# lucidrains/progen

Measured on NVIDIA H100. Metric: tokens_per_sec, higher is better.
Workload: dtype bf16

## Files before the change

progen_b200/csrc/attn_wgmma.cu:

```cuda
#include <cuda.h>
#include "common.cuh"
#include "tc_ptx.cuh"
#include "../../include/progen_b200.h"

namespace {

using namespace tc;

constexpr int DH = 64;
constexpr int TILE = 64;
constexpr int TILE_BYTES = TILE * DH * 2;
constexpr float LOG2E = 1.4426950408889634f;
constexpr float LN2 = 0.6931471805599453f;
constexpr int SMEM_BYTES = 1024  + 2 * TILE_BYTES + 2 * 2 * TILE_BYTES + 64;

struct Dims {
  int n, w, h;
  const float* rot_sin;
  const float* rot_cos;
};

__device__ __forceinline__ float quad_max(float v) {
  v = fmaxf(v, __shfl_xor_sync(0xffffffffu, v, 1));
  return fmaxf(v, __shfl_xor_sync(0xffffffffu, v, 2));
}
__device__ __forceinline__ float quad_sum(float v) {
  v += __shfl_xor_sync(0xffffffffu, v, 1);
  return v + __shfl_xor_sync(0xffffffffu, v, 2);
}
__device__ __forceinline__ uint32_t unrotate_pack(const Dims& dm, int pos, int jj, float d0, float d1) {
  if (dm.rot_sin) {
    const float s = __ldg(dm.rot_sin + pos * (DH / 2) + jj), c = __ldg(dm.rot_cos + pos * (DH / 2) + jj);
    const float a = d0 * c + d1 * s, b = d1 * c - d0 * s;
    d0 = a; d1 = b;
  }
  return pack_bf16x2(d0, d1);
}
template <int R> __device__ __forceinline__ void zero(float (&a)[R]) {
#pragma unroll
  for (int i = 0; i < R; ++i) a[i] = 0.f;
}
__device__ __forceinline__ void acc_to_a(uint32_t (&a)[4][4], const float (&s)[32]) {
#pragma unroll
  for (int kk = 0; kk < 4; ++kk)
#pragma unroll
    for (int i = 0; i < 4; ++i) a[kk][i] = pack_bf16x2(s[8 * kk + 2 * i], s[8 * kk + 2 * i + 1]);
}
__device__ __forceinline__ void issue_a_xt(float (&acc)[32], uint32_t a, uint32_t x) {
#pragma unroll
  for (int kk = 0; kk < 4; ++kk) wgmma_m64n64k16_ss<0>(acc, make_smem_desc<false>(a + 32 * kk), make_smem_desc<false>(x + 32 * kk));
}
__device__ __forceinline__ void issue_p_x(float (&acc)[32], const uint32_t (&p)[4][4], uint32_t x) {
#pragma unroll
  for (int kk = 0; kk < 4; ++kk) wgmma_m64n64k16_rs<1>(acc, p[kk], make_smem_desc<true>(x + 2048 * kk));
}
template <int R> __device__ __forceinline__ void mma_begin(float (&acc)[R]) {
  fence_regs(acc);
  wgmma_fence();
}
template <int R> __device__ __forceinline__ void mma_end(float (&acc)[R]) {
  wgmma_commit();
  wgmma_wait<0>();
  fence_regs(acc);
}

struct Smem {
  uint32_t fixed0, fixed1, ring, bars;
  __device__ Smem(uint8_t* raw) {
    fixed0 = (smem_u32(raw) + 1023u) & ~1023u;
    fixed1 = fixed0 + TILE_BYTES;
    ring = fixed1 + TILE_BYTES;
    bars = ring + 4 * TILE_BYTES;
  }
  __device__ uint32_t a(int st) const { return ring + st * 2 * TILE_BYTES; }
  __device__ uint32_t b(int st) const { return a(st) + TILE_BYTES; }
  __device__ uint32_t fixed_bar() const { return bars; }
  __device__ uint32_t full(int st) const { return bars + 8 + 8 * st; }
};

__device__ __forceinline__ void init_bars(const Smem& sm) {
  if (threadIdx.x == 0) {
    mbar_init(sm.fixed_bar(), 1);
    mbar_init(sm.full(0), 1);
    mbar_init(sm.full(1), 1);
    fence_barrier_init();
  }
  __syncthreads();
}

__global__ void __launch_bounds__(128) attn_fwd_wgmma_kernel(const __grid_constant__ CUtensorMap tm_qkv, bf16* __restrict__ out,
                                                             float* __restrict__ lse, const Dims dm) {
  extern __shared__ uint8_t smem_raw[];
  const Smem sm(smem_raw);
  const int tid = threadIdx.x, lane = tid & 31, warp = tid >> 5;
  const int g = lane >> 2, t4 = lane & 3;
  const int b = blockIdx.z, hh = blockIdx.y;
  const int q0 = blockIdx.x * TILE, win = q0 / dm.w, i0 = q0 % dm.w;
  const int I = dm.h * DH;
  const int row0 = b * dm.n;
  const int nprev = win > 0 ? dm.w / TILE : 0;
  const int ntiles = nprev + (i0 + TILE) / TILE;
  auto key_pos = [&](int kt) { return kt < nprev ? (win - 1) * dm.w + kt * TILE : win * dm.w + (kt - nprev) * TILE; };
  auto issue = [&](int kt, int st) {
    mbar_expect_tx(sm.full(st), 2 * TILE_BYTES);
    tma_load_2d(sm.a(st), &tm_qkv, sm.full(st), I + hh * DH, row0 + key_pos(kt));
    tma_load_2d(sm.b(st), &tm_qkv, sm.full(st), 2 * I + hh * DH, row0 + key_pos(kt));
  };
  init_bars(sm);
  if (tid == 0) {
    prefetch_tensormap(&tm_qkv);
    mbar_expect_tx(sm.fixed_bar(), TILE_BYTES);
    tma_load_2d(sm.fixed0, &tm_qkv, sm.fixed_bar(), hh * DH, row0 + q0);
    for (int kt = 0; kt < 2 && kt < ntiles; ++kt) issue(kt, kt);
  }

  const float sc = 0.125f  * LOG2E;
  float m_run[2], l_run[2];
  m_run[0] = m_run[1] = (win == 0) ? 0.f : -INFINITY;
  l_run[0] = l_run[1] = (win == 0) ? (float)dm.w : 0.f;
  float o[32];
  zero(o);
  const int qi_lo = i0 + warp * 16;
  mbar_wait(sm.fixed_bar(), 0);

  for (int kt = 0; kt < ntiles; ++kt) {
    const int st = kt & 1;
    mbar_wait(sm.full(st), (kt >> 1) & 1);
    float s[32];
    zero(s);
    mma_begin(s);
    issue_a_xt(s, sm.fixed0, sm.a(st));
    mma_end(s);
    const int c0 = (kt - nprev) * TILE;
    const bool need_mask = kt >= nprev && c0 + TILE - 1 > qi_lo;
    float tmax[2] = {-INFINITY, -INFINITY};
#pragma unroll
    for (int i = 0; i < 32; ++i) {
      float v = s[i] * sc;
      if (need_mask) {
        const int kj = c0 + 8 * (i >> 2) + 2 * t4 + (i & 1);
        const int qi = qi_lo + g + (((i >> 1) & 1) << 3);
        if (kj > qi) v = -INFINITY;
      }
      s[i] = v;
      tmax[(i >> 1) & 1] = fmaxf(tmax[(i >> 1) & 1], v);
    }
    float corr[2], rsum[2] = {0.f, 0.f};
#pragma unroll
    for (int r = 0; r < 2; ++r) {
      const float mn = fmaxf(m_run[r], quad_max(tmax[r]));
      corr[r] = exp2f(m_run[r] - mn);
      m_run[r] = mn;
    }
#pragma unroll
    for (int i = 0; i < 32; ++i) {
      const float p = exp2f(s[i] - m_run[(i >> 1) & 1]);
      s[i] = p;
      rsum[(i >> 1) & 1] += p;
    }
#pragma unroll
    for (int r = 0; r < 2; ++r) l_run[r] = l_run[r] * corr[r] + quad_sum(rsum[r]);
#pragma unroll
    for (int i = 0; i < 32; ++i) o[i] *= corr[(i >> 1) & 1];
    uint32_t pa[4][4];
    acc_to_a(pa, s);
    mma_begin(o);
    issue_p_x(o, pa, sm.b(st));
    mma_end(o);
    __syncthreads();
    if (tid == 0 && kt + 2 < ntiles) {
      fence_proxy_async();
      issue(kt + 2, st);
    }
  }
#pragma unroll
  for (int r = 0; r < 2; ++r) {
    const long long t = (long long)row0 + q0 + warp * 16 + g + 8 * r;
    const float inv = 1.f / l_run[r];
    bf16* op = out + t * I + hh * DH + 2 * t4;
#pragma unroll
    for (int j = 0; j < 8; ++j)
      *reinterpret_cast<uint32_t*>(op + 8 * j) = pack_bf16x2(o[4 * j + 2 * r] * inv, o[4 * j + 2 * r + 1] * inv);
    if (t4 == 0) lse[t * dm.h + hh] = m_run[r] * LN2 + logf(l_run[r]);
  }
}

__global__ void __launch_bounds__(128) attn_bwd_dq_wgmma_kernel(const __grid_constant__ CUtensorMap tm_qkv,
                                                                const __grid_constant__ CUtensorMap tm_do,
                                                                const bf16* __restrict__ out, const bf16* __restrict__ dout,
                                                                const float* __restrict__ lse, float* __restrict__ delta,
                                                                bf16* __restrict__ dqkv, const Dims dm) {
  extern __shared__ uint8_t smem_raw[];
  const Smem sm(smem_raw);
  const int tid = threadIdx.x, lane = tid & 31, warp = tid >> 5;
  const int g = lane >> 2, t4 = lane & 3;
  const int b = blockIdx.z, hh = blockIdx.y;
  const int q0 = blockIdx.x * TILE, win = q0 / dm.w, i0 = q0 % dm.w;
  const int I = dm.h * DH;
  const long long ld = 3LL * I;
  const int row0 = b * dm.n;
  const int nprev = win > 0 ? dm.w / TILE : 0;
  const int ntiles = nprev + (i0 + TILE) / TILE;
  auto key_pos = [&](int kt) { return kt < nprev ? (win - 1) * dm.w + kt * TILE : win * dm.w + (kt - nprev) * TILE; };
  auto issue = [&](int kt, int st) {
    mbar_expect_tx(sm.full(st), 2 * TILE_BYTES);
    tma_load_2d(sm.a(st), &tm_qkv, sm.full(st), I + hh * DH, row0 + key_pos(kt));
    tma_load_2d(sm.b(st), &tm_qkv, sm.full(st), 2 * I + hh * DH, row0 + key_pos(kt));
  };
  init_bars(sm);
  if (tid == 0) {
    prefetch_tensormap(&tm_qkv);
    prefetch_tensormap(&tm_do);
    mbar_expect_tx(sm.fixed_bar(), 2 * TILE_BYTES);
    tma_load_2d(sm.fixed0, &tm_qkv, sm.fixed_bar(), hh * DH, row0 + q0);
    tma_load_2d(sm.fixed1, &tm_do, sm.fixed_bar(), hh * DH, row0 + q0);
    for (int kt = 0; kt < 2 && kt < ntiles; ++kt) issue(kt, kt);
  }

  const float scale = 0.125f ;
  const float sc = scale * LOG2E;
  float L2[2], Dl[2];
#pragma unroll
  for (int r = 0; r < 2; ++r) {
    const long long t = (long long)row0 + q0 + warp * 16 + g + 8 * r;
    L2[r] = lse[t * dm.h + hh] * LOG2E;
    float acc = 0.f;
#pragma unroll
    for (int j = 0; j < 8; ++j) {
      const uint32_t ov = *reinterpret_cast<const uint32_t*>(out + t * I + hh * DH + 8 * j + 2 * t4);
      const uint32_t dv = *reinterpret_cast<const uint32_t*>(dout + t * I + hh * DH + 8 * j + 2 * t4);
      const float2 fo = __bfloat1622float2(*reinterpret_cast<const __nv_bfloat162*>(&ov));
      const float2 fd = __bfloat1622float2(*reinterpret_cast<const __nv_bfloat162*>(&dv));
      acc += fo.x * fd.x + fo.y * fd.y;
    }
    Dl[r] = quad_sum(acc);
    if (t4 == 0) delta[t * dm.h + hh] = Dl[r];
  }
  float dq[32];
  zero(dq);
  const int qi_lo = i0 + warp * 16;
  mbar_wait(sm.fixed_bar(), 0);

  for (int kt = 0; kt < ntiles; ++kt) {
    const int st = kt & 1;
    mbar_wait(sm.full(st), (kt >> 1) & 1);
    float s[32], dp[32];
    zero(s);
    zero(dp);
    fence_regs(dp);
    mma_begin(s);
    issue_a_xt(s, sm.fixed0, sm.a(st));
    issue_a_xt(dp, sm.fixed1, sm.b(st));
    mma_end(s);
    fence_regs(dp);
    const int c0 = (kt - nprev) * TILE;
    const bool need_mask = kt >= nprev && c0 + TILE - 1 > qi_lo;
#pragma unroll
    for (int i = 0; i < 32; ++i) {
      const int r = (i >> 1) & 1;
      float p = exp2f(s[i] * sc - L2[r]);
      if (need_mask) {
        const int kj = c0 + 8 * (i >> 2) + 2 * t4 + (i & 1);
        const int qi = qi_lo + g + (r << 3);
        if (kj > qi) p = 0.f;
      }
      s[i] = p * (dp[i] - Dl[r]) * scale;
    }
    uint32_t dsa[4][4];
    acc_to_a(dsa, s);
    mma_begin(dq);
    issue_p_x(dq, dsa, sm.a(st));
    mma_end(dq);
    __syncthreads();
    if (tid == 0 && kt + 2 < ntiles) {
      fence_proxy_async();
      issue(kt + 2, st);
    }
  }
#pragma unroll
  for (int r = 0; r < 2; ++r) {
    const int pos = q0 + warp * 16 + g + 8 * r;
    bf16* op = dqkv + ((long long)row0 + pos) * ld + hh * DH + 2 * t4;
#pragma unroll
    for (int j = 0; j < 8; ++j)
      *reinterpret_cast<uint32_t*>(op + 8 * j) = unrotate_pack(dm, pos, 4 * j + t4, dq[4 * j + 2 * r], dq[4 * j + 2 * r + 1]);
  }
}

__global__ void __launch_bounds__(128) attn_bwd_dkv_wgmma_kernel(const __grid_constant__ CUtensorMap tm_qkv,
                                                                 const __grid_constant__ CUtensorMap tm_do,
                                                                 const float* __restrict__ lse, const float* __restrict__ delta,
                                                                 bf16* __restrict__ dqkv, const Dims dm) {
  extern __shared__ uint8_t smem_raw[];
  const Smem sm(smem_raw);
  const int tid = threadIdx.x, lane = tid & 31, warp = tid >> 5;
  const int g = lane >> 2, t4 = lane & 3;
  const int b = blockIdx.z, hh = blockIdx.y;
  const int k0 = blockIdx.x * TILE, win = k0 / dm.w, j0 = k0 % dm.w;
  const int I = dm.h * DH;
  const long long ld = 3LL * I;
  const int row0 = b * dm.n;
  const int nwin = dm.n / dm.w;
  const int nown = (dm.w - j0) / TILE;
  const int nnext = (win + 1 < nwin) ? dm.w / TILE : 0;
  const int ntiles = nown + nnext;
  auto q_pos = [&](int qt) { return qt < nown ? win * dm.w + j0 + qt * TILE : (win + 1) * dm.w + (qt - nown) * TILE; };
  auto issue = [&](int qt, int st) {
    mbar_expect_tx(sm.full(st), 2 * TILE_BYTES);
    tma_load_2d(sm.a(st), &tm_qkv, sm.full(st), hh * DH, row0 + q_pos(qt));
    tma_load_2d(sm.b(st), &tm_do, sm.full(st), hh * DH, row0 + q_pos(qt));
  };
  init_bars(sm);
  if (tid == 0) {
    prefetch_tensormap(&tm_qkv);
    prefetch_tensormap(&tm_do);
    mbar_expect_tx(sm.fixed_bar(), 2 * TILE_BYTES);
    tma_load_2d(sm.fixed0, &tm_qkv, sm.fixed_bar(), I + hh * DH, row0 + k0);
    tma_load_2d(sm.fixed1, &tm_qkv, sm.fixed_bar(), 2 * I + hh * DH, row0 + k0);
    for (int qt = 0; qt < 2 && qt < ntiles; ++qt) issue(qt, qt);
  }

  const float scale = 0.125f ;
  const float sc = scale * LOG2E;
  float dk[32], dv[32];
  zero(dk);
  zero(dv);
  const int kj_lo = j0 + warp * 16;
  mbar_wait(sm.fixed_bar(), 0);

  for (int qt = 0; qt < ntiles; ++qt) {
    const int st = qt & 1;
    const int qp = q_pos(qt);
    float Lq[16], Dq[16];
#pragma unroll
    for (int j = 0; j < 8; ++j)
#pragma unroll
      for (int c = 0; c < 2; ++c) {
        const long long t = (long long)row0 + qp + 8 * j + 2 * t4 + c;
        Lq[2 * j + c] = __ldg(lse + t * dm.h + hh) * LOG2E;
        Dq[2 * j + c] = __ldg(delta + t * dm.h + hh);
      }
    mbar_wait(sm.full(st), (qt >> 1) & 1);
    float s[32], dp[32];
    zero(s);
    zero(dp);
    fence_regs(dp);
    mma_begin(s);
    issue_a_xt(s, sm.fixed0, sm.a(st));
    issue_a_xt(dp, sm.fixed1, sm.b(st));
    mma_end(s);
    fence_regs(dp);
    const bool own = qt < nown;
    const int c0 = j0 + qt * TILE;
    const bool need_mask = own && c0 < kj_lo + 15;
#pragma unroll
    for (int i = 0; i < 32; ++i) {
      const int col = 8 * (i >> 2) + 2 * t4 + (i & 1);
      const int ci = 2 * (i >> 2) + (i & 1);
      float p = exp2f(s[i] * sc - Lq[ci]);
      if (need_mask) {
        const int qi = c0 + col;
        const int kj = kj_lo + g + (((i >> 1) & 1) << 3);
        if (kj > qi) p = 0.f;
      }
      dp[i] = p * (dp[i] - Dq[ci]) * scale;
      s[i] = p;
    }
    uint32_t pa[4][4], dsa[4][4];
    acc_to_a(pa, s);
    acc_to_a(dsa, dp);
    fence_regs(dk);
    mma_begin(dv);
    issue_p_x(dv, pa, sm.b(st));
    issue_p_x(dk, dsa, sm.a(st));
    mma_end(dv);
    fence_regs(dk);
    __syncthreads();
    if (tid == 0 && qt + 2 < ntiles) {
      fence_proxy_async();
      issue(qt + 2, st);
    }
  }
#pragma unroll
  for (int r = 0; r < 2; ++r) {
    const int pos = k0 + warp * 16 + g + 8 * r;
    bf16* pk = dqkv + ((long long)row0 + pos) * ld + I + hh * DH + 2 * t4;
    bf16* pv = pk + I;
#pragma unroll
    for (int j = 0; j < 8; ++j) {
      *reinterpret_cast<uint32_t*>(pk + 8 * j) = unrotate_pack(dm, pos, 4 * j + t4, dk[4 * j + 2 * r], dk[4 * j + 2 * r + 1]);
      *reinterpret_cast<uint32_t*>(pv + 8 * j) = unrotate_pack(dm, pos, 4 * j + t4, dv[4 * j + 2 * r], dv[4 * j + 2 * r + 1]);
    }
  }
}

template <typename K> int prepare(K kern) {
  static bool done = false;
  if (!done) {
    PG_CUDA(cudaFuncSetAttribute(kern, cudaFuncAttributeMaxDynamicSharedMemorySize, SMEM_BYTES));
    done = true;
  }
  return PROGEN_OK;
}

int check_dims(const void* qkv, int B, int seq_len, int window, int heads, int dim_head, bool full_windows) {
  PG_CHECK_ARG(qkv != nullptr && B > 0 && heads > 0 && dim_head == DH && window % TILE == 0 && seq_len > 0 &&
               seq_len % (full_windows ? window : TILE) == 0);
  PG_CHECK_ARG((long long)B * seq_len < (1ll << 31));
  return PROGEN_OK;
}

}

extern "C" {

int progen_local_attn_fwd_tc(const void* qkv, void* out, float* lse, int B, int seq_len, int window, int heads, int dim_head,
                             void* stream) {
  int rc = check_dims(qkv, B, seq_len, window, heads, dim_head, false);
  if (rc) return rc;
  const int I = heads * DH;
  const uint64_t T = (uint64_t)B * seq_len;
  CUtensorMap tm;
  if ((rc = pg_tensor_map_2d_bf16(qkv, 3ull * I, T, 3ull * I, DH, TILE, &tm))) return rc;
  if ((rc = prepare(attn_fwd_wgmma_kernel))) return rc;
  const Dims dm{seq_len, window, heads, nullptr, nullptr};
  attn_fwd_wgmma_kernel<<<dim3(seq_len / TILE, heads, B), 128, SMEM_BYTES, (cudaStream_t)stream>>>(tm, (bf16*)out, lse, dm);
  PG_LAUNCH_CHECK();
  return PROGEN_OK;
}

int progen_local_attn_bwd_tc(const void* qkv, const void* out, const void* dout, const float* lse, void* dqkv, float* delta,
                             const float* rot_sin, const float* rot_cos, int B, int seq_len, int window, int heads, int dim_head,
                             void* stream) {
  int rc = check_dims(qkv, B, seq_len, window, heads, dim_head, true);
  if (rc) return rc;
  const int I = heads * DH;
  const uint64_t T = (uint64_t)B * seq_len;
  CUtensorMap tq, tdo;
  if ((rc = pg_tensor_map_2d_bf16(qkv, 3ull * I, T, 3ull * I, DH, TILE, &tq))) return rc;
  if ((rc = pg_tensor_map_2d_bf16(dout, (uint64_t)I, T, (uint64_t)I, DH, TILE, &tdo))) return rc;
  if ((rc = prepare(attn_bwd_dq_wgmma_kernel))) return rc;
  if ((rc = prepare(attn_bwd_dkv_wgmma_kernel))) return rc;
  const Dims dm{seq_len, window, heads, rot_sin, rot_cos};
  const dim3 grid(seq_len / TILE, heads, B);
  cudaStream_t s = (cudaStream_t)stream;
  attn_bwd_dq_wgmma_kernel<<<grid, 128, SMEM_BYTES, s>>>(tq, tdo, (const bf16*)out, (const bf16*)dout, lse, delta, (bf16*)dqkv, dm);
  PG_LAUNCH_CHECK();
  attn_bwd_dkv_wgmma_kernel<<<grid, 128, SMEM_BYTES, s>>>(tq, tdo, lse, delta, (bf16*)dqkv, dm);
  PG_LAUNCH_CHECK();
  return PROGEN_OK;
}

}
```

Baseline: 955,800.

## Software-pipeline dK/dV backward kernel with three-stage TMA ring

Restructures the attention dK/dV backward kernel so the score and dP WGMMAs for tile qt are issued together with the dV/dK accumulation WGMMAs for tile qt-1. The softmax-gradient math then overlaps with in-flight tensor-core work instead of waiting on each MMA group serially. The TMA ring for this kernel grows from two stages to three, with shared-memory size now computed per kernel. This raises register pressure from keeping pa/dsa live across iterations and uses more shared memory, which may reduce occupancy.

```diff
diff --git a/progen_b200/csrc/attn_wgmma.cu b/progen_b200/csrc/attn_wgmma.cu
--- a/progen_b200/csrc/attn_wgmma.cu
+++ b/progen_b200/csrc/attn_wgmma.cu
@@ -12,7 +12,8 @@
 constexpr int TILE_BYTES = TILE * DH * 2;
 constexpr float LOG2E = 1.4426950408889634f;
 constexpr float LN2 = 0.6931471805599453f;
-constexpr int SMEM_BYTES = 1024  + 2 * TILE_BYTES + 2 * 2 * TILE_BYTES + 64;
+constexpr int smem_bytes(int stages) { return 1024  + 2 * TILE_BYTES + stages * 2 * TILE_BYTES + 64; }
+constexpr int DKV_STAGES = 3;
 
 struct Dims {
   int n, w, h;
@@ -66,11 +67,11 @@
 
 struct Smem {
   uint32_t fixed0, fixed1, ring, bars;
-  __device__ Smem(uint8_t* raw) {
+  __device__ Smem(uint8_t* raw, int stages) {
     fixed0 = (smem_u32(raw) + 1023u) & ~1023u;
     fixed1 = fixed0 + TILE_BYTES;
     ring = fixed1 + TILE_BYTES;
-    bars = ring + 4 * TILE_BYTES;
+    bars = ring + stages * 2 * TILE_BYTES;
   }
   __device__ uint32_t a(int st) const { return ring + st * 2 * TILE_BYTES; }
   __device__ uint32_t b(int st) const { return a(st) + TILE_BYTES; }
@@ -78,11 +79,10 @@
   __device__ uint32_t full(int st) const { return bars + 8 + 8 * st; }
 };
 
-__device__ __forceinline__ void init_bars(const Smem& sm) {
+__device__ __forceinline__ void init_bars(const Smem& sm, int stages) {
   if (threadIdx.x == 0) {
     mbar_init(sm.fixed_bar(), 1);
-    mbar_init(sm.full(0), 1);
-    mbar_init(sm.full(1), 1);
+    for (int st = 0; st < stages; ++st) mbar_init(sm.full(st), 1);
     fence_barrier_init();
   }
   __syncthreads();
@@ -91,7 +91,7 @@
 __global__ void __launch_bounds__(128) attn_fwd_wgmma_kernel(const __grid_constant__ CUtensorMap tm_qkv, bf16* __restrict__ out,
                                                              float* __restrict__ lse, const Dims dm) {
   extern __shared__ uint8_t smem_raw[];
-  const Smem sm(smem_raw);
+  const Smem sm(smem_raw, 2);
   const int tid = threadIdx.x, lane = tid & 31, warp = tid >> 5;
   const int g = lane >> 2, t4 = lane & 3;
   const int b = blockIdx.z, hh = blockIdx.y;
@@ -106,7 +106,7 @@
     tma_load_2d(sm.a(st), &tm_qkv, sm.full(st), I + hh * DH, row0 + key_pos(kt));
     tma_load_2d(sm.b(st), &tm_qkv, sm.full(st), 2 * I + hh * DH, row0 + key_pos(kt));
   };
-  init_bars(sm);
+  init_bars(sm, 2);
   if (tid == 0) {
     prefetch_tensormap(&tm_qkv);
     mbar_expect_tx(sm.fixed_bar(), TILE_BYTES);
@@ -191,7 +191,7 @@
                                                                 const float* __restrict__ lse, float* __restrict__ delta,
                                                                 bf16* __restrict__ dqkv, const Dims dm) {
   extern __shared__ uint8_t smem_raw[];
-  const Smem sm(smem_raw);
+  const Smem sm(smem_raw, 2);
   const int tid = threadIdx.x, lane = tid & 31, warp = tid >> 5;
   const int g = lane >> 2, t4 = lane & 3;
   const int b = blockIdx.z, hh = blockIdx.y;
@@ -207,7 +207,7 @@
     tma_load_2d(sm.a(st), &tm_qkv, sm.full(st), I + hh * DH, row0 + key_pos(kt));
     tma_load_2d(sm.b(st), &tm_qkv, sm.full(st), 2 * I + hh * DH, row0 + key_pos(kt));
   };
-  init_bars(sm);
+  init_bars(sm, 2);
   if (tid == 0) {
     prefetch_tensormap(&tm_qkv);
     prefetch_tensormap(&tm_do);
@@ -291,8 +291,9 @@
                                                                  const __grid_constant__ CUtensorMap tm_do,
                                                                  const float* __restrict__ lse, const float* __restrict__ delta,
                                                                  bf16* __restrict__ dqkv, const Dims dm) {
+  constexpr int NS = DKV_STAGES;
   extern __shared__ uint8_t smem_raw[];
-  const Smem sm(smem_raw);
+  const Smem sm(smem_raw, NS);
   const int tid = threadIdx.x, lane = tid & 31, warp = tid >> 5;
   const int g = lane >> 2, t4 = lane & 3;
   const int b = blockIdx.z, hh = blockIdx.y;
@@ -310,14 +311,14 @@
     tma_load_2d(sm.a(st), &tm_qkv, sm.full(st), hh * DH, row0 + q_pos(qt));
     tma_load_2d(sm.b(st), &tm_do, sm.full(st), hh * DH, row0 + q_pos(qt));
   };
-  init_bars(sm);
+  init_bars(sm, NS);
   if (tid == 0) {
     prefetch_tensormap(&tm_qkv);
     prefetch_tensormap(&tm_do);
     mbar_expect_tx(sm.fixed_bar(), 2 * TILE_BYTES);
     tma_load_2d(sm.fixed0, &tm_qkv, sm.fixed_bar(), I + hh * DH, row0 + k0);
     tma_load_2d(sm.fixed1, &tm_qkv, sm.fixed_bar(), 2 * I + hh * DH, row0 + k0);
-    for (int qt = 0; qt < 2 && qt < ntiles; ++qt) issue(qt, qt);
+    for (int qt = 0; qt < NS && qt < ntiles; ++qt) issue(qt, qt);
   }
 
   const float scale = 0.125f ;
@@ -326,12 +327,9 @@
   zero(dk);
   zero(dv);
   const int kj_lo = j0 + warp * 16;
-  mbar_wait(sm.fixed_bar(), 0);
-
-  for (int qt = 0; qt < ntiles; ++qt) {
-    const int st = qt & 1;
+  float Lq[16], Dq[16];
+  auto load_lse_delta = [&](int qt) {
     const int qp = q_pos(qt);
-    float Lq[16], Dq[16];
 #pragma unroll
     for (int j = 0; j < 8; ++j)
 #pragma unroll
@@ -340,16 +338,26 @@
         Lq[2 * j + c] = __ldg(lse + t * dm.h + hh) * LOG2E;
         Dq[2 * j + c] = __ldg(delta + t * dm.h + hh);
       }
-    mbar_wait(sm.full(st), (qt >> 1) & 1);
-    float s[32], dp[32];
+  };
+  auto scores = [&](float (&s)[32], float (&dp)[32], int st) {
     zero(s);
     zero(dp);
+    fence_regs(s);
     fence_regs(dp);
-    mma_begin(s);
+    fence_regs(dk);
+    fence_regs(dv);
+    wgmma_fence();
     issue_a_xt(s, sm.fixed0, sm.a(st));
     issue_a_xt(dp, sm.fixed1, sm.b(st));
-    mma_end(s);
-    fence_regs(dp);
+    wgmma_commit();
+  };
+  uint32_t pa[4][4], dsa[4][4];
+  auto accumulate = [&](int st) {
+    issue_p_x(dv, pa, sm.b(st));
+    issue_p_x(dk, dsa, sm.a(st));
+    wgmma_commit();
+  };
+  auto grad = [&](float (&s)[32], float (&dp)[32], int qt) {
     const bool own = qt < nown;
     const int c0 = j0 + qt * TILE;
     const bool need_mask = own && c0 < kj_lo + 15;
@@ -366,21 +374,50 @@
       dp[i] = p * (dp[i] - Dq[ci]) * scale;
       s[i] = p;
     }
-    uint32_t pa[4][4], dsa[4][4];
+  };
+  mbar_wait(sm.fixed_bar(), 0);
+
+  {
+    load_lse_delta(0);
+    mbar_wait(sm.full(0), 0);
+    float s[32], dp[32];
+    scores(s, dp, 0);
+    wgmma_wait<0>();
+    fence_regs(s);
+    fence_regs(dp);
+    grad(s, dp, 0);
     acc_to_a(pa, s);
     acc_to_a(dsa, dp);
+  }
+  for (int qt = 1; qt < ntiles; ++qt) {
+    const int st = qt % NS, prev = (qt - 1) % NS;
+    load_lse_delta(qt);
+    mbar_wait(sm.full(st), (qt / NS) & 1);
+    float s[32], dp[32];
+    scores(s, dp, st);
+    accumulate(prev);
+    wgmma_wait<1>();
+    fence_regs(s);
+    fence_regs(dp);
+    grad(s, dp, qt);
+    wgmma_wait<0>();
     fence_regs(dk);
-    mma_begin(dv);
-    issue_p_x(dv, pa, sm.b(st));
-    issue_p_x(dk, dsa, sm.a(st));
-    mma_end(dv);
-    fence_regs(dk);
+    fence_regs(dv);
     __syncthreads();
-    if (tid == 0 && qt + 2 < ntiles) {
+    if (tid == 0 && qt - 1 + NS < ntiles) {
       fence_proxy_async();
-      issue(qt + 2, st);
-    }
-  }
+      issue(qt - 1 + NS, prev);
+    }
+    acc_to_a(pa, s);
+    acc_to_a(dsa, dp);
+  }
+  fence_regs(dk);
+  fence_regs(dv);
+  wgmma_fence();
+  accumulate((ntiles - 1) % NS);
+  wgmma_wait<0>();
+  fence_regs(dk);
+  fence_regs(dv);
 #pragma unroll
   for (int r = 0; r < 2; ++r) {
     const int pos = k0 + warp * 16 + g + 8 * r;
@@ -394,10 +431,10 @@
   }
 }
 
-template <typename K> int prepare(K kern) {
+template <typename K> int prepare(K kern, int bytes) {
   static bool done = false;
   if (!done) {
-    PG_CUDA(cudaFuncSetAttribute(kern, cudaFuncAttributeMaxDynamicSharedMemorySize, SMEM_BYTES));
+    PG_CUDA(cudaFuncSetAttribute(kern, cudaFuncAttributeMaxDynamicSharedMemorySize, bytes));
     done = true;
   }
   return PROGEN_OK;
@@ -422,9 +459,9 @@
   const uint64_t T = (uint64_t)B * seq_len;
   CUtensorMap tm;
   if ((rc = pg_tensor_map_2d_bf16(qkv, 3ull * I, T, 3ull * I, DH, TILE, &tm))) return rc;
-  if ((rc = prepare(attn_fwd_wgmma_kernel))) return rc;
+  if ((rc = prepare(attn_fwd_wgmma_kernel, smem_bytes(2)))) return rc;
   const Dims dm{seq_len, window, heads, nullptr, nullptr};
-  attn_fwd_wgmma_kernel<<<dim3(seq_len / TILE, heads, B), 128, SMEM_BYTES, (cudaStream_t)stream>>>(tm, (bf16*)out, lse, dm);
+  attn_fwd_wgmma_kernel<<<dim3(seq_len / TILE, heads, B), 128, smem_bytes(2), (cudaStream_t)stream>>>(tm, (bf16*)out, lse, dm);
   PG_LAUNCH_CHECK();
   return PROGEN_OK;
 }
@@ -439,14 +476,14 @@
   CUtensorMap tq, tdo;
   if ((rc = pg_tensor_map_2d_bf16(qkv, 3ull * I, T, 3ull * I, DH, TILE, &tq))) return rc;
   if ((rc = pg_tensor_map_2d_bf16(dout, (uint64_t)I, T, (uint64_t)I, DH, TILE, &tdo))) return rc;
-  if ((rc = prepare(attn_bwd_dq_wgmma_kernel))) return rc;
-  if ((rc = prepare(attn_bwd_dkv_wgmma_kernel))) return rc;
+  if ((rc = prepare(attn_bwd_dq_wgmma_kernel, smem_bytes(2)))) return rc;
+  if ((rc = prepare(attn_bwd_dkv_wgmma_kernel, smem_bytes(DKV_STAGES)))) return rc;
   const Dims dm{seq_len, window, heads, rot_sin, rot_cos};
   const dim3 grid(seq_len / TILE, heads, B);
   cudaStream_t s = (cudaStream_t)stream;
-  attn_bwd_dq_wgmma_kernel<<<grid, 128, SMEM_BYTES, s>>>(tq, tdo, (const bf16*)out, (const bf16*)dout, lse, delta, (bf16*)dqkv, dm);
+  attn_bwd_dq_wgmma_kernel<<<grid, 128, smem_bytes(2), s>>>(tq, tdo, (const bf16*)out, (const bf16*)dout, lse, delta, (bf16*)dqkv, dm);
   PG_LAUNCH_CHECK();
-  attn_bwd_dkv_wgmma_kernel<<<grid, 128, SMEM_BYTES, s>>>(tq, tdo, lse, delta, (bf16*)dqkv, dm);
+  attn_bwd_dkv_wgmma_kernel<<<grid, 128, smem_bytes(DKV_STAGES), s>>>(tq, tdo, lse, delta, (bf16*)dqkv, dm);
   PG_LAUNCH_CHECK();
   return PROGEN_OK;
 }
```

Result: no change. 960,400, median of 6 (+0.5%).
